# vlongle/pixie

Measured on NVIDIA H100. Metric: unet_voxels_per_s, higher is better.
Workload: dtype fp16e5 (U-Net, fp32 accumulate) + f32 (MPM)

## Files before the change

### pixie_b200/csrc/conv3d_igemm.cu

```cuda
#include "conv3d_igemm.cuh"
#include "ptx.cuh"

#include <algorithm>
#include <cmath>
#include <cstdio>
#include <cstring>

#include <cuda_fp8.h>

namespace pixie {

using namespace ptx;

namespace {

constexpr int kMaxWStages = 4;
constexpr int kMaxSStages = 8;
constexpr int kConsumerWarps = 8;
constexpr int kProducerWarp = 8;

struct SmemCtrl {
    uint64_t wfull[kMaxWStages];
    uint64_t wempty[kMaxWStages];
    uint64_t sfull[kMaxSStages];
    uint64_t sempty[kMaxSStages];
    int abort_flag;
};

constexpr int kCtlBarrierBytes = 512;
constexpr int kCmChunk = 16;
constexpr int kCmStageLd = 68;
constexpr int kCmStageFloats = kCmChunk * kCmStageLd;
constexpr int kStatsMaxC = 256;

struct TileCoord {
    int nb, d0, h0, w0, n0, ph_begin, ph_end, split, tde;
};

__device__ __forceinline__ TileCoord decode_tile(const ConvKernelParams& p, int wi) {
    TileCoord t;
    unsigned rest = (unsigned)wi;
    if (p.split_k == 1) {
        t.split = 0; t.ph_begin = 0; t.ph_end = p.n_phases;
    } else {
        const unsigned sk = (unsigned)p.split_k;
        t.split = (int)(rest % sk);
        rest /= sk;
        t.ph_begin = (int)(((unsigned)t.split * (unsigned)p.n_phases) / sk);
// ... 62 lines not shown
};

struct PendingStages {
    int s = -1, w = -1;
    __device__ __forceinline__ void release(SmemCtrl* ctl, int lane) {
        if (lane == 0) {
            if (s >= 0) mbar_arrive(&ctl->sempty[s]);
            if (w >= 0) mbar_arrive(&ctl->wempty[w]);
        }
        s = -1; w = -1;
    }
};

struct ConvStats {
    float* rows;
    int nb = -1;
    double tot_s = 0.0, tot_q = 0.0;

    __device__ __forceinline__ void flush(const ConvKernelParams& p, int lane) {
        if (p.stats_scalar) {
#pragma unroll
            for (int off = 16; off >= 1; off >>= 1) {
                tot_s += __shfl_xor_sync(0xffffffffu, tot_s, off);
                tot_q += __shfl_xor_sync(0xffffffffu, tot_q, off);
            }
            if (lane == 0) {
                atomicAdd(p.stats + (size_t)nb * p.Cout * 2, tot_s);
                atomicAdd(p.stats + (size_t)nb * p.Cout * 2 + 1, tot_q);
            }
            tot_s = 0.0; tot_q = 0.0;
            return;
        }
        asm volatile("bar.sync 1, 256;" ::: "memory");
        for (int ch = threadIdx.x; ch < p.Cout; ch += 256) {
            atomicAdd(p.stats + ((size_t)nb * p.Cout + ch) * 2, (double)rows[ch]);
            atomicAdd(p.stats + ((size_t)nb * p.Cout + ch) * 2 + 1, (double)rows[p.stats_ld + ch]);
            rows[ch] = 0.f;
            rows[p.stats_ld + ch] = 0.f;
        }
        asm volatile("bar.sync 1, 256;" ::: "memory");
    }
    __device__ __forceinline__ void enter(const ConvKernelParams& p, int item_nb, int lane) {
        if (nb != item_nb) {
            if (nb >= 0) flush(p, lane);
            nb = item_nb;
        }
    }
};

struct ConvSmem {
    uint8_t* w;
    uint8_t* s;
    SmemCtrl* ctl;
    float* stage;
    float* stats;
};

__device__ __forceinline__ ConvSmem conv_prologue(const ConvKernelParams& p, int stage_floats, int n_threads) {
    extern __shared__ __align__(1024) uint8_t smem_raw[];
    uint8_t* smem = reinterpret_cast<uint8_t*>(
        (reinterpret_cast<uintptr_t>(smem_raw) + 1023) & ~static_cast<uintptr_t>(1023));
    ConvSmem m;
    m.w = smem;
    m.s = smem + (size_t)p.w_stages * p.w_stage_bytes;
    m.ctl = reinterpret_cast<SmemCtrl*>(m.s + (size_t)p.s_stages * p.s_stage_bytes);
    m.stage = reinterpret_cast<float*>(reinterpret_cast<uint8_t*>(m.ctl) + kCtlBarrierBytes);
    m.stats = m.stage + stage_floats;
    const bool smem_misaligned = (p.smem_slack == 0) && (smem != smem_raw);

    if (threadIdx.x == 0) {
        for (int i = 0; i < kMaxWStages; ++i) { mbar_init(&m.ctl->wfull[i], 1); mbar_init(&m.ctl->wempty[i], kConsumerWarps); }
        for (int i = 0; i < kMaxSStages; ++i) { mbar_init(&m.ctl->sfull[i], 1); mbar_init(&m.ctl->sempty[i], kConsumerWarps); }
        m.ctl->abort_flag = smem_misaligned ? 1 : 0;
        fence_barrier_init();
    }
    if ((threadIdx.x >> 5) == kProducerWarp && (threadIdx.x & 31) == 0) {
        for (int i = 0; i < kConvMaxSrc; ++i) prefetch_tmap(&p.tmA[i]);
        prefetch_tmap(&p.tmB);
    }
    if (p.stats != nullptr && !p.stats_scalar)
        for (int i = threadIdx.x; i < 2 * p.stats_ld; i += n_threads) m.stats[i] = 0.f;
    __syncthreads();
    return m;
}

__device__ __forceinline__ void conv_report_abort(const ConvKernelParams& p, const SmemCtrl* ctl) {
    __syncthreads();
    if (threadIdx.x == 0 && ctl->abort_flag && p.err_flag) atomicExch(p.err_flag, 1 + (int)blockIdx.x);
}

template <int BN, int TD>
__device__ __forceinline__ int issue_slab(float (&acc)[TD][BN / 2], uint32_t a_addr, uint32_t w_addr, int pl, int d_min, int d_max,
                                          int n_kd, int n_kh, int TW, bool f8) {
    int groups = 0;
#pragma unroll
    for (int d = 0; d < TD; ++d) {
// ... 44 lines not shown
                    wring.advance(p.w_stages);
                }
                ok = mbar_wait(&ctl->sempty[sring.stage], sring.parity ^ 1, abort_flag);
                if (!ok) break;
                if (elect_one()) {
                    mbar_expect_tx(&ctl->sfull[sring.stage], slab_bytes);
                    tma_load_5d(s_smem + (size_t)sring.stage * p.s_stage_bytes, tm, &ctl->sfull[sring.stage], (int)P.c0, cw, ch,
                                cd + pl * p.stride, t.nb);
                }
                sring.advance(p.s_stages);
            }
        }
    }
}

}

template <int BN, int TD>
__global__ void __launch_bounds__(kConvThreads, 1)
conv3d_igemm_kernel(const __grid_constant__ ConvKernelParams p) {
    const ConvSmem sm = conv_prologue(p, 0, kConvThreads);
    SmemCtrl* ctl = sm.ctl;
    volatile int* abort_flag = &ctl->abort_flag;
    const int warp = threadIdx.x >> 5;
    const int lane = threadIdx.x & 31;
    const int total_items = conv_work_items(p.NB, p.tiles_d, p.tiles_h, p.tiles_w, p.n_tiles, p.split_k);
    const bool do_stats = p.stats != nullptr;
    const bool scalar_stats = do_stats && p.stats_scalar;

    if (warp == kProducerWarp) {
        produce_tiles<kWholePhase>(p, ctl, sm.w, sm.s, abort_flag, total_items);
    } else {
        const int g = warp >> 2, wq = warp & 3;
        float acc[TD][BN / 2];
        RingPos wring, sring;
        const uint32_t w_base0 = smem_u32(sm.w), s_base0 = smem_u32(sm.s) + (uint32_t)(g * 64 * 128);
        bool ok = true;
        const long long DHW = (long long)p.D * p.H * p.W;
        ConvStats stats{sm.stats};
        int th2[2], tw2[2];
#pragma unroll
        for (int r2 = 0; r2 < 2; ++r2) {
            const int r = g * 64 + wq * 16 + (lane >> 2) + 8 * r2;
            th2[r2] = r / p.TW; tw2[r2] = r % p.TW;
        }
        const int cq = (lane & 3) * 2;

        for (int wi = blockIdx.x; wi < total_items && ok; wi += gridDim.x) {
            const TileCoord t = decode_tile(p, wi);
#pragma unroll
            for (int d = 0; d < TD; ++d)
#pragma unroll
                for (int j = 0; j < BN / 2; ++j) acc[d][j] = 0.f;
            PendingStages pend;
// ... 113 lines not shown
                            const int ch = t.n0 + j8 * 8 + cq + e;
                            if (lane < 4 && ch < p.Cout) {
                                atomicAdd(stats.rows + ch, s);
                                atomicAdd(stats.rows + p.stats_ld + ch, q2);
                            }
                        }
                }
            }
        }
        if (do_stats && stats.nb >= 0 && ok) stats.flush(p, lane);
    }

    conv_report_abort(p, ctl);
}

template <int NV>
__global__ void __launch_bounds__(kConvCmThreads, 1)
conv3d_igemm_cm_kernel(const __grid_constant__ ConvKernelParams p) {
    constexpr int TW = NV == 64 ? 8 : 16;
    const ConvSmem sm = conv_prologue(p, 2 * kCmStageFloats, kConvCmThreads);
    SmemCtrl* ctl = sm.ctl;
    volatile int* abort_flag = &ctl->abort_flag;
    const int warp = threadIdx.x >> 5;
    const int lane = threadIdx.x & 31;
    const int total_items = conv_work_items(p.NB, p.tiles_d, p.tiles_h, p.tiles_w, p.n_tiles, p.split_k);
    const bool do_stats = p.stats != nullptr;
    const bool scalar_stats = do_stats && p.stats_scalar;

    if (warp >= kProducerWarp) {
        setmaxnreg_dec<NV == 256 ? 40 : 56>();
        if (warp == kProducerWarp) produce_tiles<1>(p, ctl, sm.w, sm.s, abort_flag, total_items);
    } else {
        setmaxnreg_inc<NV == 256 ? 232 : 216>();
        const int g = warp >> 2, wq = warp & 3, wt = threadIdx.x & 127;
        float acc[NV / 2];
        RingPos wring, sring;
        const uint32_t w_base0 = smem_u32(sm.w), s_base0 = smem_u32(sm.s);
        bool ok = true;
        ConvStats stats{sm.stats};
        const int q4 = wt & 15, vr = wt >> 4;
        float* stage = sm.stage + g * kCmStageFloats;

        for (int wi = blockIdx.x; wi < total_items && ok; wi += gridDim.x) {
            const TileCoord t = decode_tile(p, wi);
#pragma unroll
            for (int j = 0; j < NV / 2; ++j) acc[j] = 0.f;
            const bool has_plane = g < t.tde;
            PendingStages pend;
            int prev_f8 = -1;
            for (int ph = t.ph_begin; ph < t.ph_end && ok; ++ph) {
                const ConvPhase P = p.phases[ph];
                const int n_kd = P.n_kd, n_kh = P.n_kh;
                const bool f8 = P.f8 != 0;
                if (prev_f8 >= 0 && prev_f8 != (int)f8) wgmma_wait<0>();
                prev_f8 = (int)f8;
                const int w0 = wring.stage;
                const int nplanes = t.tde + n_kd - 1;
                for (int pl = 0; pl < nplanes && ok; ++pl) {
                    if (pl < n_kd) {
                        ok = mbar_wait(&ctl->wfull[wring.stage], wring.parity, abort_flag);
                        if (!ok) break;
                        wring.advance(p.w_stages);
                    }
                    ok = mbar_wait(&ctl->sfull[sring.stage], sring.parity, abort_flag);
                    if (!ok) break;
                    const int kd = pl - g;
                    int groups = 0;
                    if (has_plane && kd >= 0 && kd < n_kd) {
                        int wsk = w0 + kd;
                        if (wsk >= p.w_stages) wsk -= p.w_stages;
                        const uint32_t w_addr = w_base0 + (uint32_t)(wsk * p.w_stage_bytes);
                        const uint32_t s_addr = s_base0 + (uint32_t)(sring.stage * p.s_stage_bytes);
                        for (int kh = 0; kh < n_kh; ++kh) {
                            const uint32_t a = w_addr + (uint32_t)(conv_wtile(0, 1, kh, 0) * 64 * 128);
                            const uint32_t b = s_addr + (uint32_t)(kh * TW * 128);
                            if (f8) mma_block<NV, true>(acc, a, b);
                            else mma_block<NV, false>(acc, a, b);
                            ++groups;
                        }
                    }
                    wgmma_wait_n(groups);
                    pend.release(ctl, lane);
                    pend.s = sring.stage;
                    const int kd_done = pl - t.tde + 1;
                    if (kd_done >= 0) {
                        pend.w = w0 + kd_done;
                        if (pend.w >= p.w_stages) pend.w -= p.w_stages;
                    }
                    sring.advance(p.s_stages);
                }
            }
            wgmma_wait<0>();
            pend.release(ctl, lane);
#pragma unroll
            for (int j = 0; j < NV / 2; ++j) fence_operand(acc[j]);
            if (!ok) break;

            if (do_stats) stats.enter(p, t.nb, lane);
            if (!has_plane) continue;
            const bool first_split = (t.split == 0);
            const int ch = t.n0 + 4 * q4;
            const bool ch_ok = ch < p.Cout;
            float4 bias4 = make_float4(0.f, 0.f, 0.f, 0.f);
            if (first_split && p.bias != nullptr && ch_ok)
                bias4 = make_float4(__ldg(p.bias + ch), __ldg(p.bias + ch + 1), __ldg(p.bias + ch + 2), __ldg(p.bias + ch + 3));
            const bool use_res = first_split && p.residual != nullptr;
            const long long plane_base = ((long long)t.nb * p.D + t.d0 + g) * p.H;
            float st_s[4] = {0.f, 0.f, 0.f, 0.f}, st_q[4] = {0.f, 0.f, 0.f, 0.f};
#pragma unroll
            for (int c = 0; c < NV / kCmChunk; ++c) {
#pragma unroll
                for (int jj = 0; jj < kCmChunk / 8; ++jj)
#pragma unroll
                    for (int r2 = 0; r2 < 2; ++r2)
#pragma unroll
                        for (int e = 0; e < 2; ++e) {
                            const int row = wq * 16 + (lane >> 2) + 8 * r2, v = jj * 8 + (lane & 3) * 2 + e;
                            stage[v * kCmStageLd + row] = acc[(c * (kCmChunk / 8) + jj) * 4 + r2 * 2 + e];
                        }
                asm volatile("bar.sync %0, 128;" ::"r"(2 + g) : "memory");
#pragma unroll
                for (int k = 0; k < kCmChunk / 8; ++k) {
                    const int v = vr + 8 * k, vt = c * kCmChunk + v;
                    const int hh = t.h0 + vt / TW, ww = t.w0 + vt % TW;
                    float4 x = *reinterpret_cast<const float4*>(stage + v * kCmStageLd + 4 * q4);
                    if (ch_ok && hh < p.H && ww < p.W) {
                        const long long base = ((plane_base + hh) * p.W + ww) * p.out_ld + p.out_c0 + ch;
                        x.x += bias4.x; x.y += bias4.y; x.z += bias4.z; x.w += bias4.w;
                        if (use_res) {
                            const float4 rv = __ldg(reinterpret_cast<const float4*>(p.residual + base));
                            x.x += rv.x; x.y += rv.y; x.z += rv.z; x.w += rv.w;
                        }
                        if (p.atomic_out) red_add_v4(p.out + base, x.x, x.y, x.z, x.w);
                        else *reinterpret_cast<float4*>(p.out + base) = x;
                        st_s[0] += x.x; st_s[1] += x.y; st_s[2] += x.z; st_s[3] += x.w;
                        st_q[0] = fmaf(x.x, x.x, st_q[0]); st_q[1] = fmaf(x.y, x.y, st_q[1]);
                        st_q[2] = fmaf(x.z, x.z, st_q[2]); st_q[3] = fmaf(x.w, x.w, st_q[3]);
                    }
                }
                asm volatile("bar.sync %0, 128;" ::"r"(2 + g) : "memory");
            }
            if (do_stats) {
                if (scalar_stats) {
                    stats.tot_s += (double)(st_s[0] + st_s[1] + st_s[2] + st_s[3]);
                    stats.tot_q += (double)(st_q[0] + st_q[1] + st_q[2] + st_q[3]);
                } else {
#pragma unroll
                    for (int i = 0; i < 4; ++i) {
                        st_s[i] += __shfl_xor_sync(0xffffffffu, st_s[i], 16);
                        st_q[i] += __shfl_xor_sync(0xffffffffu, st_q[i], 16);
                    }
                    if (lane < 16 && ch_ok) {
#pragma unroll
                        for (int i = 0; i < 4; ++i) {
                            atomicAdd(stats.rows + ch + i, st_s[i]);
                            atomicAdd(stats.rows + p.stats_ld + ch + i, st_q[i]);
                        }
                    }
                }
            }
        }
        if (do_stats && stats.nb >= 0 && ok) stats.flush(p, lane);
    }

    conv_report_abort(p, ctl);
}


int conv_k_total(const ConvDesc& d) {
    int k = 0;
    for (const auto& s : d.segs) k += s.ks * s.ks * s.ks * d.srcs[s.src].C;
    return k;
}

struct SrcSlot { int src; int n_kh; };
// ... 144 lines not shown
        CUresult r = enc(&p.tmA[i], CU_TENSOR_MAP_DATA_TYPE_FLOAT16, 5, (void*)s.ptr, gdim, gstr, box, estr,
                         CU_TENSOR_MAP_INTERLEAVE_NONE, CU_TENSOR_MAP_SWIZZLE_128B,
                         CU_TENSOR_MAP_L2_PROMOTION_L2_256B, CU_TENSOR_MAP_FLOAT_OOB_FILL_NONE);
        if (r != CUDA_SUCCESS) { snprintf(err, errlen, "cuTensorMapEncodeTiled(A%zu) failed: %d", i, (int)r); return 1; }
    }
    for (size_t i = slots.size(); i < (size_t)kConvMaxSrc; ++i) p.tmA[i] = p.tmA[0];
    return 0;
}

int conv_plan_retarget(const ConvDesc& d, ConvPlan& plan, char* err, int errlen) {
    PFN_encodeTiled enc = get_encode_fn();
    if (!enc) { snprintf(err, errlen, "cuTensorMapEncodeTiled unavailable"); return 1; }
    return encode_a_maps(d, plan.p, enc, err, errlen);
}

static const char* cm_geometry(const ConvDesc& d, int sms, int max_kh, ConvKernelParams& p) {
    int nv = d.nv;
    if (nv && nv != 64 && nv != 128 && nv != 256) return "bad nv";
    if (!nv) {
        double best = -1.0;
        for (int v : {256, 128, 64}) {
            if (v != 64 && d.W < 16) continue;
            const int tw = v == 64 ? 8 : 16, th = v / tw;
            const int tx = (d.W + tw - 1) / tw, ty = (d.H + th - 1) / th;
            const long long tiles = conv_work_items(d.NB, (d.D + 1) / 2, ty, tx, (d.Cout_pad + 63) / 64, 1);
            const long long rounds = (tiles + sms - 1) / sms;
            const double sc = (double)tiles / (double)(rounds * sms) * (double)d.W * d.H / (double)(tx * tw * ty * th) *
                              std::pow(0.93, v == 256 ? 0 : v == 128 ? 1 : 2);
            if (sc > best) { best = sc; nv = v; }
        }
    }
    p.TW = nv == 64 ? 8 : 16;
    p.TH = nv / p.TW;
    p.TD = 2;
    p.block_n = 64;
    p.w_stage_bytes = max_kh * p.block_n * 128;
    return nullptr;
}

static bool cm_stages(const ConvKernelParams& p, int max_kd, int avail, int& ws, int& ss) {
    ws = std::max(2, max_kd);
    if (ws * p.w_stage_bytes + 2 * p.s_stage_bytes > avail) return false;
    ss = std::min(std::min(kMaxSStages, 6), (avail - ws * p.w_stage_bytes) / p.s_stage_bytes);
    ws = std::min(kMaxWStages, (avail - ss * p.s_stage_bytes) / p.w_stage_bytes);
    return true;
}
// ... 54 lines not shown
    int max_taps = 1, max_kh = 1, max_kd = 1;
    bool any3 = false;
    for (const auto& P : phases) {
        max_taps = std::max(max_taps, P.n_kh * P.n_kd);
        max_kh = std::max(max_kh, (int)P.n_kh);
        max_kd = std::max(max_kd, (int)P.n_kd);
        any3 |= (P.n_kh == 3);
    }

    int dev = 0, sms = 132;
    cudaGetDevice(&dev);
    cudaDeviceGetAttribute(&sms, cudaDevAttrMultiProcessorCount, dev);

    plan.channel_major = d.Cout >= 64 && d.Cout % 4 == 0 && !d.out_planar && out_ld % 4 == 0 && d.out_c0 % 4 == 0 &&
                         reinterpret_cast<uintptr_t>(d.out) % 16 == 0 && reinterpret_cast<uintptr_t>(d.residual) % 16 == 0;
    const char* bad = plan.channel_major ? cm_geometry(d, sms, max_kh, p) : vm_geometry(d, sms, any3, max_taps, p);
    if (bad) return fail(bad);
    p.n_tiles = (d.Cout_pad + p.block_n - 1) / p.block_n;
    p.tiles_w = (d.W + p.TW - 1) / p.TW;
    p.tiles_h = (d.H + p.TH - 1) / p.TH;
    p.tiles_d = (d.D + p.TD - 1) / p.TD;

    const int items = conv_work_items(d.NB, p.tiles_d, p.tiles_h, p.tiles_w, p.n_tiles, 1);
    int split = d.split_k;
    if (split <= 0) {
        split = 1;
        while (items * split < 120 && split * 2 <= p.n_phases && split < 64) split *= 2;
    }
    split = std::max(1, std::min(split, p.n_phases));
    if ((long long)p.n_phases * (split + 1) >= (1ll << 31)) return fail("too many phases for the split-K bookkeeping");
    p.split_k = split;
    p.atomic_out = split > 1;
    plan.needs_zero = split > 1;

    for (size_t i = 0; i < slots.size(); ++i) p.slab_rows[i] = p.TW * (p.TH + slots[i].n_kh - 1);
    int max_rows = 0;
    for (size_t i = 0; i < slots.size(); ++i) max_rows = std::max(max_rows, p.slab_rows[i]);
    p.s_stage_bytes = max_rows * 128;
    plan.fused_stats = d.stats != nullptr && split == 1 && d.Cout <= kStatsMaxC && !d.out_planar;
    p.stats_ld = (d.Cout + 31) / 32 * 32;
    const int stats_bytes = plan.fused_stats ? 2 * p.stats_ld * 4 : 0;
    const int ctl_core = kCtlBarrierBytes + (plan.channel_major ? 2 * kCmStageFloats * 4 : 0) + stats_bytes;
    auto plan_stages = [&](int slack, int& ws, int& ss) {
        const int avail = 227 * 1024 - ctl_core - slack;
        return plan.channel_major ? cm_stages(p, max_kd, avail, ws, ss) : vm_stages(p, avail, ws, ss);
    };
    int ws1 = 0, ss1 = 0, ws0 = 0, ss0 = 0;
    const bool ok1 = plan_stages(1024, ws1, ss1), ok0 = plan_stages(0, ws0, ss0);
    if (!ok0) return fail("tile does not fit in shared memory");
    if (ok1 && ws1 >= ws0 && ss1 >= ss0) { p.smem_slack = 1024; p.w_stages = ws1; p.s_stages = ss1; }
    else { p.smem_slack = 0; p.w_stages = ws0; p.s_stages = ss0; }
    const int ctl_bytes = ctl_core + p.smem_slack;
    plan.smem_bytes = p.w_stages * p.w_stage_bytes + p.s_stages * p.s_stage_bytes + ctl_bytes;

    if (encode_a_maps(d, p, enc, err, errlen)) return 1;
    {
// ... 10 lines not shown

    if (cudaMalloc(&plan.d_phases, phases.size() * sizeof(ConvPhase)) != cudaSuccess) return fail("cudaMalloc phases");
    cudaMemcpy(plan.d_phases, phases.data(), phases.size() * sizeof(ConvPhase), cudaMemcpyHostToDevice);
    p.phases = plan.d_phases;

    p.bias = d.bias; p.residual = d.residual; p.out = d.out;
    p.out_ld = out_ld; p.out_c0 = d.out_c0; p.out_planar = d.out_planar;
    p.err_flag = d_err_flag;
    p.stats = plan.fused_stats ? d.stats : nullptr;
    p.stats_scalar = d.stats_scalar ? 1 : 0;
    plan.out_item_bytes = d.out_planar ? (size_t)d.Cout * d.D * d.H * d.W * 4
                                       : (size_t)d.D * d.H * d.W * p.out_ld * 4;

    plan.grid = std::min(items * split, sms);

    plan.kernel = plan.channel_major ? conv_cm_kernel_for(p.TH * p.TW) : conv_kernel_for(p.block_n, p.TD);
    plan.threads = plan.channel_major ? kConvCmThreads : kConvThreads;
    if (cudaFuncSetAttribute(plan.kernel, cudaFuncAttributeMaxDynamicSharedMemorySize, 227 * 1024) != cudaSuccess)
        return fail("cudaFuncSetAttribute(max dynamic smem)");
    return 0;
}

void conv_plan_destroy(ConvPlan& plan) {
    if (plan.d_phases) cudaFree(plan.d_phases);
    plan.d_phases = nullptr;
}

int conv_plan_launch(const ConvPlan& plan, int nb, cudaStream_t stream) {
    if (nb < 1 || nb > plan.p.NB) return (int)cudaErrorInvalidValue;
    ConvKernelParams p = plan.p;
    p.NB = nb;
// ... 8 lines not shown
```

### pixie_b200/csrc/conv3d_igemm.cuh

```cuda
#pragma once
#include <cuda.h>
#include <cuda_runtime.h>
#include <cuda_fp16.h>
#include <cstdint>
#include <vector>

namespace pixie {

constexpr int kConvMaxSrc = 8;
constexpr int kF8Shift = 6;
constexpr int kConvThreads = 288;
constexpr int kConvCmThreads = 384;

struct ConvPhase {
    int8_t src;
    int8_t dw;
    int8_t dh0;
    int8_t dd0;
    int8_t n_kh;
    int8_t n_kd;
    int16_t c0;
    int32_t wtile_base;
    int32_t f8;
};
// ... 53 lines not shown
    struct Seg { int src; int ks; int wlo = 0; int f8 = 0; int lo = 0; };
    std::vector<ConvSrc> srcs;
    std::vector<Seg> segs;
    const __half* weights = nullptr;
    int Cout_pad = 0;
    const float* bias = nullptr;
    const float* residual = nullptr;
    float* out = nullptr;
    int out_ld = 0, out_c0 = 0, out_planar = 0;
    double* stats = nullptr;
    bool stats_scalar = false;
    int split_k = 1;
    int block_n = 0;
    int td = 0;
    int nv = 0;
};

int conv_k_total(const ConvDesc& d);

std::vector<ConvPhase> conv_build_phases(const ConvDesc& d);

void conv_pack_weights(const ConvDesc& d, const std::vector<const float*>& seg_weights,
                       const std::vector<int>& seg_cin_real, std::vector<__half>& packed);

struct ConvPlan {
    ConvKernelParams p{};
    ConvPhase* d_phases = nullptr;
    ConvKernelFn kernel = nullptr;
    bool channel_major = false;
    int threads = 0;
    int grid = 0;
    int smem_bytes = 0;
    bool needs_zero = false;
    bool fused_stats = false;
    size_t out_item_bytes = 0;
};

int conv_plan_create(const ConvDesc& d, int* d_err_flag, ConvPlan& plan, char* err, int errlen);
void conv_plan_destroy(ConvPlan& plan);
int conv_plan_launch(const ConvPlan& plan, int nb, cudaStream_t stream);
int conv_plan_retarget(const ConvDesc& d, ConvPlan& plan, char* err, int errlen);
}
```

### pixie_b200/csrc/ptx.cuh

```cuda
#pragma once
#include <cstdint>
#include <cuda_runtime.h>

namespace pixie {
namespace ptx {

__device__ __forceinline__ uint32_t smem_u32(const void* p) {
    return static_cast<uint32_t>(__cvta_generic_to_shared(p));
}

__device__ __forceinline__ bool elect_one() {
    uint32_t pred = 0;
    asm volatile(
        "{\n\t"
        ".reg .pred P;\n\t"
        "elect.sync _|P, 0xffffffff;\n\t"
        "selp.u32 %0, 1, 0, P;\n\t"
        "}\n"
        : "=r"(pred));
    return pred != 0;
}

__device__ __forceinline__ void mbar_init(uint64_t* bar, uint32_t count) {
    asm volatile("mbarrier.init.shared::cta.b64 [%0], %1;" ::"r"(smem_u32(bar)), "r"(count));
// ... 146 lines not shown
        : "+f"(d[0]), "+f"(d[1]), "+f"(d[2]), "+f"(d[3]), "+f"(d[4]), "+f"(d[5]), "+f"(d[6]), "+f"(d[7]), "+f"(d[8]), "+f"(d[9]), "+f"(d[10]), "+f"(d[11]), "+f"(d[12]), "+f"(d[13]), "+f"(d[14]), "+f"(d[15]), "+f"(d[16]), "+f"(d[17]), "+f"(d[18]), "+f"(d[19]), "+f"(d[20]), "+f"(d[21]), "+f"(d[22]), "+f"(d[23]), "+f"(d[24]), "+f"(d[25]), "+f"(d[26]), "+f"(d[27]), "+f"(d[28]), "+f"(d[29]), "+f"(d[30]), "+f"(d[31]), "+f"(d[32]), "+f"(d[33]), "+f"(d[34]), "+f"(d[35]), "+f"(d[36]), "+f"(d[37]), "+f"(d[38]), "+f"(d[39]), "+f"(d[40]), "+f"(d[41]), "+f"(d[42]), "+f"(d[43]), "+f"(d[44]), "+f"(d[45]), "+f"(d[46]), "+f"(d[47]), "+f"(d[48]), "+f"(d[49]), "+f"(d[50]), "+f"(d[51]), "+f"(d[52]), "+f"(d[53]), "+f"(d[54]), "+f"(d[55]), "+f"(d[56]), "+f"(d[57]), "+f"(d[58]), "+f"(d[59]), "+f"(d[60]), "+f"(d[61]), "+f"(d[62]), "+f"(d[63])
        : "l"(da), "l"(db), "r"(1));
}
__device__ __forceinline__ void wgmma_e5m2_n256(float* d, uint64_t da, uint64_t db) {
    asm volatile(
        "{\n\t.reg .pred p;\n\tsetp.ne.b32 p, %130, 0;\n\t"
        "wgmma.mma_async.sync.aligned.m64n256k32.f32.e5m2.e5m2 "
        "{%0, %1, %2, %3, %4, %5, %6, %7, %8, %9, %10, %11, %12, %13, %14, %15, %16, %17, %18, %19, %20, %21, %22, %23, %24, %25, %26, %27, %28, %29, %30, %31, %32, %33, %34, %35, %36, %37, %38, %39, %40, %41, %42, %43, %44, %45, %46, %47, %48, %49, %50, %51, %52, %53, %54, %55, %56, %57, %58, %59, %60, %61, %62, %63, %64, %65, %66, %67, %68, %69, %70, %71, %72, %73, %74, %75, %76, %77, %78, %79, %80, %81, %82, %83, %84, %85, %86, %87, %88, %89, %90, %91, %92, %93, %94, %95, %96, %97, %98, %99, %100, %101, %102, %103, %104, %105, %106, %107, %108, %109, %110, %111, %112, %113, %114, %115, %116, %117, %118, %119, %120, %121, %122, %123, %124, %125, %126, %127}, %128, %129, p, 1, 1;\n\t}\n"
        : "+f"(d[0]), "+f"(d[1]), "+f"(d[2]), "+f"(d[3]), "+f"(d[4]), "+f"(d[5]), "+f"(d[6]), "+f"(d[7]), "+f"(d[8]), "+f"(d[9]), "+f"(d[10]), "+f"(d[11]), "+f"(d[12]), "+f"(d[13]), "+f"(d[14]), "+f"(d[15]), "+f"(d[16]), "+f"(d[17]), "+f"(d[18]), "+f"(d[19]), "+f"(d[20]), "+f"(d[21]), "+f"(d[22]), "+f"(d[23]), "+f"(d[24]), "+f"(d[25]), "+f"(d[26]), "+f"(d[27]), "+f"(d[28]), "+f"(d[29]), "+f"(d[30]), "+f"(d[31]), "+f"(d[32]), "+f"(d[33]), "+f"(d[34]), "+f"(d[35]), "+f"(d[36]), "+f"(d[37]), "+f"(d[38]), "+f"(d[39]), "+f"(d[40]), "+f"(d[41]), "+f"(d[42]), "+f"(d[43]), "+f"(d[44]), "+f"(d[45]), "+f"(d[46]), "+f"(d[47]), "+f"(d[48]), "+f"(d[49]), "+f"(d[50]), "+f"(d[51]), "+f"(d[52]), "+f"(d[53]), "+f"(d[54]), "+f"(d[55]), "+f"(d[56]), "+f"(d[57]), "+f"(d[58]), "+f"(d[59]), "+f"(d[60]), "+f"(d[61]), "+f"(d[62]), "+f"(d[63]), "+f"(d[64]), "+f"(d[65]), "+f"(d[66]), "+f"(d[67]), "+f"(d[68]), "+f"(d[69]), "+f"(d[70]), "+f"(d[71]), "+f"(d[72]), "+f"(d[73]), "+f"(d[74]), "+f"(d[75]), "+f"(d[76]), "+f"(d[77]), "+f"(d[78]), "+f"(d[79]), "+f"(d[80]), "+f"(d[81]), "+f"(d[82]), "+f"(d[83]), "+f"(d[84]), "+f"(d[85]), "+f"(d[86]), "+f"(d[87]), "+f"(d[88]), "+f"(d[89]), "+f"(d[90]), "+f"(d[91]), "+f"(d[92]), "+f"(d[93]), "+f"(d[94]), "+f"(d[95]), "+f"(d[96]), "+f"(d[97]), "+f"(d[98]), "+f"(d[99]), "+f"(d[100]), "+f"(d[101]), "+f"(d[102]), "+f"(d[103]), "+f"(d[104]), "+f"(d[105]), "+f"(d[106]), "+f"(d[107]), "+f"(d[108]), "+f"(d[109]), "+f"(d[110]), "+f"(d[111]), "+f"(d[112]), "+f"(d[113]), "+f"(d[114]), "+f"(d[115]), "+f"(d[116]), "+f"(d[117]), "+f"(d[118]), "+f"(d[119]), "+f"(d[120]), "+f"(d[121]), "+f"(d[122]), "+f"(d[123]), "+f"(d[124]), "+f"(d[125]), "+f"(d[126]), "+f"(d[127])
        : "l"(da), "l"(db), "r"(1));
}
template <int N>
__device__ __forceinline__ void setmaxnreg_dec() { asm volatile("setmaxnreg.dec.sync.aligned.u32 %0;" ::"n"(N)); }
template <int N>
__device__ __forceinline__ void setmaxnreg_inc() { asm volatile("setmaxnreg.inc.sync.aligned.u32 %0;" ::"n"(N)); }


__device__ __forceinline__ void cp_async_16(void* smem_dst, const void* gmem_src) {
    asm volatile("cp.async.cg.shared.global [%0], [%1], 16;" ::"r"(smem_u32(smem_dst)), "l"(gmem_src) : "memory");
}
__device__ __forceinline__ void cp_async_commit() { asm volatile("cp.async.commit_group;" ::: "memory"); }
template <int N>
__device__ __forceinline__ void cp_async_wait() { asm volatile("cp.async.wait_group %0;" ::"n"(N) : "memory"); }

__device__ __forceinline__ void red_add_v2(float* addr, float a, float b) {
    asm volatile("red.global.add.v2.f32 [%0], {%1, %2};" ::"l"(addr), "f"(a), "f"(b) : "memory");
}
__device__ __forceinline__ void red_add_v4(float* addr, float a, float b, float c, float d) {
    asm volatile("red.global.add.v4.f32 [%0], {%1, %2, %3, %4};" ::"l"(addr), "f"(a), "f"(b),
                 "f"(c), "f"(d)
// ... 16 lines not shown
```

Measured before the change: 16.02 million.

## Add ping-pong warpgroup schedule for channel-major conv3d implicit GEMM

Adds a channel-major conv kernel in which the two consumer warpgroups alternate work items. Each accumulates both depth planes of a 128-voxel tile, and named barriers hand over the turn so one group's epilogue overlaps the other's WGMMA mainloop. The mainloop, epilogue chunking and stats code are factored into shared helpers, and stats get per-group smem rows and barriers. The host geometry picker scores the ping-pong option with a penalty factor, and split-K is disabled for it. The cost is more register pressure (two accumulators) and extra synchronization complexity.

```diff
diff --git a/pixie_b200/csrc/conv3d_igemm.cu b/pixie_b200/csrc/conv3d_igemm.cu
--- a/pixie_b200/csrc/conv3d_igemm.cu
+++ b/pixie_b200/csrc/conv3d_igemm.cu
@@ -32,6 +32,7 @@
 constexpr int kCmStageLd = 68;
 constexpr int kCmStageFloats = kCmChunk * kCmStageLd;
 constexpr int kStatsMaxC = 256;
+constexpr double kPingPongGain = 0.75;
 
 struct TileCoord {
     int nb, d0, h0, w0, n0, ph_begin, ph_end, split, tde;
@@ -124,6 +125,7 @@
 
 struct ConvStats {
     float* rows;
+    int bar, n_thr, tid;
     int nb = -1;
     double tot_s = 0.0, tot_q = 0.0;
 
@@ -141,14 +143,14 @@
             tot_s = 0.0; tot_q = 0.0;
             return;
         }
-        asm volatile("bar.sync 1, 256;" ::: "memory");
-        for (int ch = threadIdx.x; ch < p.Cout; ch += 256) {
+        named_bar_sync(bar, n_thr);
+        for (int ch = tid; ch < p.Cout; ch += n_thr) {
             atomicAdd(p.stats + ((size_t)nb * p.Cout + ch) * 2, (double)rows[ch]);
             atomicAdd(p.stats + ((size_t)nb * p.Cout + ch) * 2 + 1, (double)rows[p.stats_ld + ch]);
             rows[ch] = 0.f;
             rows[p.stats_ld + ch] = 0.f;
         }
-        asm volatile("bar.sync 1, 256;" ::: "memory");
+        named_bar_sync(bar, n_thr);
     }
     __device__ __forceinline__ void enter(const ConvKernelParams& p, int item_nb, int lane) {
         if (nb != item_nb) {
@@ -166,7 +168,8 @@
     float* stats;
 };
 
-__device__ __forceinline__ ConvSmem conv_prologue(const ConvKernelParams& p, int stage_floats, int n_threads) {
+__device__ __forceinline__ ConvSmem conv_prologue(const ConvKernelParams& p, int stage_floats, int n_threads,
+                                                  int consumer_warps = kConsumerWarps, int stats_sets = 1) {
     extern __shared__ __align__(1024) uint8_t smem_raw[];
     uint8_t* smem = reinterpret_cast<uint8_t*>(
         (reinterpret_cast<uintptr_t>(smem_raw) + 1023) & ~static_cast<uintptr_t>(1023));
@@ -179,8 +182,8 @@
     const bool smem_misaligned = (p.smem_slack == 0) && (smem != smem_raw);
 
     if (threadIdx.x == 0) {
-        for (int i = 0; i < kMaxWStages; ++i) { mbar_init(&m.ctl->wfull[i], 1); mbar_init(&m.ctl->wempty[i], kConsumerWarps); }
-        for (int i = 0; i < kMaxSStages; ++i) { mbar_init(&m.ctl->sfull[i], 1); mbar_init(&m.ctl->sempty[i], kConsumerWarps); }
+        for (int i = 0; i < kMaxWStages; ++i) { mbar_init(&m.ctl->wfull[i], 1); mbar_init(&m.ctl->wempty[i], consumer_warps); }
+        for (int i = 0; i < kMaxSStages; ++i) { mbar_init(&m.ctl->sfull[i], 1); mbar_init(&m.ctl->sempty[i], consumer_warps); }
         m.ctl->abort_flag = smem_misaligned ? 1 : 0;
         fence_barrier_init();
     }
@@ -189,7 +192,7 @@
         prefetch_tmap(&p.tmB);
     }
     if (p.stats != nullptr && !p.stats_scalar)
-        for (int i = threadIdx.x; i < 2 * p.stats_ld; i += n_threads) m.stats[i] = 0.f;
+        for (int i = threadIdx.x; i < 2 * p.stats_ld * stats_sets; i += n_threads) m.stats[i] = 0.f;
     __syncthreads();
     return m;
 }
@@ -264,6 +267,171 @@
     }
 }
 
+
+
+template <int NV, int NP>
+__device__ __forceinline__ bool cm_mainloop(const ConvKernelParams& p, SmemCtrl* ctl, volatile int* abort_flag,
+                                            const TileCoord& t, float (&acc)[NP][NV / 2], int d_first, uint32_t w_base0,
+                                            uint32_t s_base0, RingPos& wring, RingPos& sring, PendingStages& pend, int lane) {
+    constexpr int TW = NV == 64 ? 8 : 16;
+#pragma unroll
+    for (int d = 0; d < NP; ++d)
+#pragma unroll
+        for (int j = 0; j < NV / 2; ++j) acc[d][j] = 0.f;
+    bool ok = true;
+    int prev_f8 = -1;
+    for (int ph = t.ph_begin; ph < t.ph_end && ok; ++ph) {
+        const ConvPhase P = p.phases[ph];
+        const int n_kd = P.n_kd, n_kh = P.n_kh;
+        const bool f8 = P.f8 != 0;
+        if (prev_f8 >= 0 && prev_f8 != (int)f8) wgmma_wait<0>();
+        prev_f8 = (int)f8;
+        const int w0 = wring.stage;
+        const int nplanes = t.tde + n_kd - 1;
+        for (int pl = 0; pl < nplanes && ok; ++pl) {
+            if (pl < n_kd) {
+                ok = mbar_wait(&ctl->wfull[wring.stage], wring.parity, abort_flag);
+                if (!ok) break;
+                wring.advance(p.w_stages);
+            }
+            ok = mbar_wait(&ctl->sfull[sring.stage], sring.parity, abort_flag);
+            if (!ok) break;
+            int groups = 0;
+#pragma unroll
+            for (int d = 0; d < NP; ++d) {
+                const int kd = pl - d_first - d;
+                if (d_first + d < t.tde && kd >= 0 && kd < n_kd) {
+                    int wsk = w0 + kd;
+                    if (wsk >= p.w_stages) wsk -= p.w_stages;
+                    const uint32_t w_addr = w_base0 + (uint32_t)(wsk * p.w_stage_bytes);
+                    const uint32_t s_addr = s_base0 + (uint32_t)(sring.stage * p.s_stage_bytes);
+                    for (int kh = 0; kh < n_kh; ++kh) {
+                        const uint32_t a = w_addr + (uint32_t)(conv_wtile(0, 1, kh, 0) * 64 * 128);
+                        const uint32_t b = s_addr + (uint32_t)(kh * TW * 128);
+                        if (f8) mma_block<NV, true>(acc[d], a, b);
+                        else mma_block<NV, false>(acc[d], a, b);
+                        ++groups;
+                    }
+                }
+            }
+            wgmma_wait_n(groups);
+            pend.release(ctl, lane);
+            pend.s = sring.stage;
+            const int kd_done = pl - t.tde + 1;
+            if (kd_done >= 0) {
+                pend.w = w0 + kd_done;
+                if (pend.w >= p.w_stages) pend.w -= p.w_stages;
+            }
+            sring.advance(p.s_stages);
+        }
+    }
+    return ok;
+}
+
+constexpr int kCmChunkRows = kCmChunk / 8;
+struct CmChunk {
+    long long base[kCmChunkRows];
+    bool ok[kCmChunkRows];
+    float4 rv[kCmChunkRows];
+};
+
+template <int NV>
+__device__ __forceinline__ CmChunk cm_chunk(const ConvKernelParams& p, const TileCoord& t, int d, int c, int wt, bool use_res) {
+    constexpr int TW = NV == 64 ? 8 : 16;
+    const int ch = t.n0 + 4 * (wt & 15), vr = wt >> 4;
+    const bool ch_ok = ch < p.Cout;
+    const long long plane_base = ((long long)t.nb * p.D + t.d0 + d) * p.H;
+    CmChunk k;
+#pragma unroll
+    for (int r = 0; r < kCmChunkRows; ++r) {
+        const int vt = c * kCmChunk + vr + 8 * r;
+        const int hh = t.h0 + vt / TW, ww = t.w0 + vt % TW;
+        k.ok[r] = ch_ok && hh < p.H && ww < p.W;
+        k.base[r] = ((plane_base + hh) * p.W + ww) * p.out_ld + p.out_c0 + ch;
+        k.rv[r] = make_float4(0.f, 0.f, 0.f, 0.f);
+    }
+    if (use_res) {
+#pragma unroll
+        for (int r = 0; r < kCmChunkRows; ++r)
+            if (k.ok[r]) k.rv[r] = __ldg(reinterpret_cast<const float4*>(p.residual + k.base[r]));
+    }
+    return k;
+}
+
+template <int NV, bool kAhead>
+__device__ __forceinline__ void cm_store_plane(const ConvKernelParams& p, const TileCoord& t, int d, const float (&acc)[NV / 2],
+                                               CmChunk cur, float* stage, int bar, int wt, float4 bias4, bool use_res,
+                                               float (&st_s)[4], float (&st_q)[4]) {
+    const int lane = wt & 31, wq = wt >> 5, q4 = wt & 15, vr = wt >> 4;
+#pragma unroll
+    for (int c = 0; c < NV / kCmChunk; ++c) {
+        CmChunk next;
+        if (kAhead && c + 1 < NV / kCmChunk) next = cm_chunk<NV>(p, t, d, c + 1, wt, use_res);
+        if (!kAhead && c > 0) cur = cm_chunk<NV>(p, t, d, c, wt, use_res);
+#pragma unroll
+        for (int jj = 0; jj < kCmChunk / 8; ++jj)
+#pragma unroll
+            for (int r2 = 0; r2 < 2; ++r2)
+#pragma unroll
+                for (int e = 0; e < 2; ++e) {
+                    const int row = wq * 16 + (lane >> 2) + 8 * r2, v = jj * 8 + (lane & 3) * 2 + e;
+                    stage[v * kCmStageLd + row] = acc[(c * (kCmChunk / 8) + jj) * 4 + r2 * 2 + e];
+                }
+        named_bar_sync(bar, 128);
+#pragma unroll
+        for (int r = 0; r < kCmChunkRows; ++r) {
+            float4 x = *reinterpret_cast<const float4*>(stage + (vr + 8 * r) * kCmStageLd + 4 * q4);
+            if (cur.ok[r]) {
+                x.x += bias4.x; x.y += bias4.y; x.z += bias4.z; x.w += bias4.w;
+                if (use_res) { x.x += cur.rv[r].x; x.y += cur.rv[r].y; x.z += cur.rv[r].z; x.w += cur.rv[r].w; }
+                if (p.atomic_out) red_add_v4(p.out + cur.base[r], x.x, x.y, x.z, x.w);
+                else *reinterpret_cast<float4*>(p.out + cur.base[r]) = x;
+                st_s[0] += x.x; st_s[1] += x.y; st_s[2] += x.z; st_s[3] += x.w;
+                st_q[0] = fmaf(x.x, x.x, st_q[0]); st_q[1] = fmaf(x.y, x.y, st_q[1]);
+                st_q[2] = fmaf(x.z, x.z, st_q[2]); st_q[3] = fmaf(x.w, x.w, st_q[3]);
+            }
+        }
+        named_bar_sync(bar, 128);
+        if (kAhead && c + 1 < NV / kCmChunk) cur = next;
+    }
+}
+
+__device__ __forceinline__ float4 cm_bias4(const ConvKernelParams& p, const TileCoord& t, int wt) {
+    const int ch = t.n0 + 4 * (wt & 15);
+    if (t.split != 0 || p.bias == nullptr || ch >= p.Cout) return make_float4(0.f, 0.f, 0.f, 0.f);
+    return make_float4(__ldg(p.bias + ch), __ldg(p.bias + ch + 1), __ldg(p.bias + ch + 2), __ldg(p.bias + ch + 3));
+}
+
+__device__ __forceinline__ void cm_add_stats(const ConvKernelParams& p, ConvStats& stats, const TileCoord& t, int wt,
+                                             float (&st_s)[4], float (&st_q)[4]) {
+    if (p.stats_scalar) {
+        stats.tot_s += (double)(st_s[0] + st_s[1] + st_s[2] + st_s[3]);
+        stats.tot_q += (double)(st_q[0] + st_q[1] + st_q[2] + st_q[3]);
+        return;
+    }
+#pragma unroll
+    for (int i = 0; i < 4; ++i) {
+        st_s[i] += __shfl_xor_sync(0xffffffffu, st_s[i], 16);
+        st_q[i] += __shfl_xor_sync(0xffffffffu, st_q[i], 16);
+    }
+    const int ch = t.n0 + 4 * (wt & 15);
+    if ((wt & 31) < 16 && ch < p.Cout) {
+#pragma unroll
+        for (int i = 0; i < 4; ++i) {
+            atomicAdd(stats.rows + ch + i, st_s[i]);
+            atomicAdd(stats.rows + p.stats_ld + ch + i, st_q[i]);
+        }
+    }
+}
+
+__device__ __forceinline__ void cm_skip_item(const ConvKernelParams& p, const TileCoord& t, RingPos& wring, RingPos& sring) {
+    for (int ph = t.ph_begin; ph < t.ph_end; ++ph) {
+        const int n_kd = p.phases[ph].n_kd;
+        for (int u = 0; u < n_kd; ++u) wring.advance(p.w_stages);
+        for (int pl = 0; pl < t.tde + n_kd - 1; ++pl) sring.advance(p.s_stages);
+    }
+}
+
 }
 
 template <int BN, int TD>
@@ -287,7 +455,7 @@
         const uint32_t w_base0 = smem_u32(sm.w), s_base0 = smem_u32(sm.s) + (uint32_t)(g * 64 * 128);
         bool ok = true;
         const long long DHW = (long long)p.D * p.H * p.W;
-        ConvStats stats{sm.stats};
+        ConvStats stats{sm.stats, 1, 256, (int)threadIdx.x};
         int th2[2], tw2[2];
 #pragma unroll
         for (int r2 = 0; r2 < 2; ++r2) {
@@ -431,10 +599,10 @@
     conv_report_abort(p, ctl);
 }
 
+
 template <int NV>
 __global__ void __launch_bounds__(kConvCmThreads, 1)
 conv3d_igemm_cm_kernel(const __grid_constant__ ConvKernelParams p) {
-    constexpr int TW = NV == 64 ? 8 : 16;
     const ConvSmem sm = conv_prologue(p, 2 * kCmStageFloats, kConvCmThreads);
     SmemCtrl* ctl = sm.ctl;
     volatile int* abort_flag = &ctl->abort_flag;
@@ -442,140 +610,100 @@
     const int lane = threadIdx.x & 31;
     const int total_items = conv_work_items(p.NB, p.tiles_d, p.tiles_h, p.tiles_w, p.n_tiles, p.split_k);
     const bool do_stats = p.stats != nullptr;
-    const bool scalar_stats = do_stats && p.stats_scalar;
 
     if (warp >= kProducerWarp) {
         setmaxnreg_dec<NV == 256 ? 40 : 56>();
         if (warp == kProducerWarp) produce_tiles<1>(p, ctl, sm.w, sm.s, abort_flag, total_items);
     } else {
         setmaxnreg_inc<NV == 256 ? 232 : 216>();
-        const int g = warp >> 2, wq = warp & 3, wt = threadIdx.x & 127;
-        float acc[NV / 2];
+        const int g = warp >> 2, wt = threadIdx.x & 127;
+        float acc[1][NV / 2];
         RingPos wring, sring;
         const uint32_t w_base0 = smem_u32(sm.w), s_base0 = smem_u32(sm.s);
         bool ok = true;
-        ConvStats stats{sm.stats};
-        const int q4 = wt & 15, vr = wt >> 4;
+        ConvStats stats{sm.stats, 1, 256, (int)threadIdx.x};
         float* stage = sm.stage + g * kCmStageFloats;
 
         for (int wi = blockIdx.x; wi < total_items && ok; wi += gridDim.x) {
             const TileCoord t = decode_tile(p, wi);
-#pragma unroll
-            for (int j = 0; j < NV / 2; ++j) acc[j] = 0.f;
-            const bool has_plane = g < t.tde;
             PendingStages pend;
-            int prev_f8 = -1;
-            for (int ph = t.ph_begin; ph < t.ph_end && ok; ++ph) {
-                const ConvPhase P = p.phases[ph];
-                const int n_kd = P.n_kd, n_kh = P.n_kh;
-                const bool f8 = P.f8 != 0;
-                if (prev_f8 >= 0 && prev_f8 != (int)f8) wgmma_wait<0>();
-                prev_f8 = (int)f8;
-                const int w0 = wring.stage;
-                const int nplanes = t.tde + n_kd - 1;
-                for (int pl = 0; pl < nplanes && ok; ++pl) {
-                    if (pl < n_kd) {
-                        ok = mbar_wait(&ctl->wfull[wring.stage], wring.parity, abort_flag);
-                        if (!ok) break;
-                        wring.advance(p.w_stages);
-                    }
-                    ok = mbar_wait(&ctl->sfull[sring.stage], sring.parity, abort_flag);
-                    if (!ok) break;
-                    const int kd = pl - g;
-                    int groups = 0;
-                    if (has_plane && kd >= 0 && kd < n_kd) {
-                        int wsk = w0 + kd;
-                        if (wsk >= p.w_stages) wsk -= p.w_stages;
-                        const uint32_t w_addr = w_base0 + (uint32_t)(wsk * p.w_stage_bytes);
-                        const uint32_t s_addr = s_base0 + (uint32_t)(sring.stage * p.s_stage_bytes);
-                        for (int kh = 0; kh < n_kh; ++kh) {
-                            const uint32_t a = w_addr + (uint32_t)(conv_wtile(0, 1, kh, 0) * 64 * 128);
-                            const uint32_t b = s_addr + (uint32_t)(kh * TW * 128);
-                            if (f8) mma_block<NV, true>(acc, a, b);
-                            else mma_block<NV, false>(acc, a, b);
-                            ++groups;
-                        }
-                    }
-                    wgmma_wait_n(groups);
-                    pend.release(ctl, lane);
-                    pend.s = sring.stage;
-                    const int kd_done = pl - t.tde + 1;
-                    if (kd_done >= 0) {
-                        pend.w = w0 + kd_done;
-                        if (pend.w >= p.w_stages) pend.w -= p.w_stages;
-                    }
-                    sring.advance(p.s_stages);
-                }
-            }
+            ok = cm_mainloop<NV, 1>(p, ctl, abort_flag, t, acc, g, w_base0, s_base0, wring, sring, pend, lane);
+            const bool use_res = t.split == 0 && p.residual != nullptr;
+            const CmChunk first = cm_chunk<NV>(p, t, g, 0, wt, use_res && ok && g < t.tde);
             wgmma_wait<0>();
             pend.release(ctl, lane);
 #pragma unroll
-            for (int j = 0; j < NV / 2; ++j) fence_operand(acc[j]);
+            for (int j = 0; j < NV / 2; ++j) fence_operand(acc[0][j]);
             if (!ok) break;
 
             if (do_stats) stats.enter(p, t.nb, lane);
-            if (!has_plane) continue;
-            const bool first_split = (t.split == 0);
-            const int ch = t.n0 + 4 * q4;
-            const bool ch_ok = ch < p.Cout;
-            float4 bias4 = make_float4(0.f, 0.f, 0.f, 0.f);
-            if (first_split && p.bias != nullptr && ch_ok)
-                bias4 = make_float4(__ldg(p.bias + ch), __ldg(p.bias + ch + 1), __ldg(p.bias + ch + 2), __ldg(p.bias + ch + 3));
-            const bool use_res = first_split && p.residual != nullptr;
-            const long long plane_base = ((long long)t.nb * p.D + t.d0 + g) * p.H;
+            if (g >= t.tde) continue;
             float st_s[4] = {0.f, 0.f, 0.f, 0.f}, st_q[4] = {0.f, 0.f, 0.f, 0.f};
-#pragma unroll
-            for (int c = 0; c < NV / kCmChunk; ++c) {
-#pragma unroll
-                for (int jj = 0; jj < kCmChunk / 8; ++jj)
-#pragma unroll
-                    for (int r2 = 0; r2 < 2; ++r2)
-#pragma unroll
-                        for (int e = 0; e < 2; ++e) {
-                            const int row = wq * 16 + (lane >> 2) + 8 * r2, v = jj * 8 + (lane & 3) * 2 + e;
-                            stage[v * kCmStageLd + row] = acc[(c * (kCmChunk / 8) + jj) * 4 + r2 * 2 + e];
-                        }
-                asm volatile("bar.sync %0, 128;" ::"r"(2 + g) : "memory");
-#pragma unroll
-                for (int k = 0; k < kCmChunk / 8; ++k) {
-                    const int v = vr + 8 * k, vt = c * kCmChunk + v;
-                    const int hh = t.h0 + vt / TW, ww = t.w0 + vt % TW;
-                    float4 x = *reinterpret_cast<const float4*>(stage + v * kCmStageLd + 4 * q4);
-                    if (ch_ok && hh < p.H && ww < p.W) {
-                        const long long base = ((plane_base + hh) * p.W + ww) * p.out_ld + p.out_c0 + ch;
-                        x.x += bias4.x; x.y += bias4.y; x.z += bias4.z; x.w += bias4.w;
-                        if (use_res) {
-                            const float4 rv = __ldg(reinterpret_cast<const float4*>(p.residual + base));
-                            x.x += rv.x; x.y += rv.y; x.z += rv.z; x.w += rv.w;
-                        }
-                        if (p.atomic_out) red_add_v4(p.out + base, x.x, x.y, x.z, x.w);
-                        else *reinterpret_cast<float4*>(p.out + base) = x;
-                        st_s[0] += x.x; st_s[1] += x.y; st_s[2] += x.z; st_s[3] += x.w;
-                        st_q[0] = fmaf(x.x, x.x, st_q[0]); st_q[1] = fmaf(x.y, x.y, st_q[1]);
-                        st_q[2] = fmaf(x.z, x.z, st_q[2]); st_q[3] = fmaf(x.w, x.w, st_q[3]);
-                    }
-                }
-                asm volatile("bar.sync %0, 128;" ::"r"(2 + g) : "memory");
-            }
-            if (do_stats) {
-                if (scalar_stats) {
-                    stats.tot_s += (double)(st_s[0] + st_s[1] + st_s[2] + st_s[3]);
-                    stats.tot_q += (double)(st_q[0] + st_q[1] + st_q[2] + st_q[3]);
-                } else {
-#pragma unroll
-                    for (int i = 0; i < 4; ++i) {
-                        st_s[i] += __shfl_xor_sync(0xffffffffu, st_s[i], 16);
-                        st_q[i] += __shfl_xor_sync(0xffffffffu, st_q[i], 16);
-                    }
-                    if (lane < 16 && ch_ok) {
-#pragma unroll
-                        for (int i = 0; i < 4; ++i) {
-                            atomicAdd(stats.rows + ch + i, st_s[i]);
-                            atomicAdd(stats.rows + p.stats_ld + ch + i, st_q[i]);
-                        }
-                    }
-                }
-            }
+            cm_store_plane<NV, true>(p, t, g, acc[0], first, stage, 2 + g, wt, cm_bias4(p, t, wt), use_res, st_s, st_q);
+            if (do_stats) cm_add_stats(p, stats, t, wt, st_s, st_q);
+        }
+        if (do_stats && stats.nb >= 0 && ok) stats.flush(p, lane);
+    }
+
+    conv_report_abort(p, ctl);
+}
+
+constexpr int kCmTurnBar = 4;
+
+__global__ void __launch_bounds__(kConvCmThreads, 1)
+conv3d_igemm_cm_pingpong_kernel(const __grid_constant__ ConvKernelParams p) {
+    constexpr int NV = 128;
+    const ConvSmem sm = conv_prologue(p, 2 * kCmStageFloats, kConvCmThreads, kConsumerWarps / 2, 2);
+    SmemCtrl* ctl = sm.ctl;
+    volatile int* abort_flag = &ctl->abort_flag;
+    const int warp = threadIdx.x >> 5;
+    const int lane = threadIdx.x & 31;
+    const int total_items = conv_work_items(p.NB, p.tiles_d, p.tiles_h, p.tiles_w, p.n_tiles, p.split_k);
+    const bool do_stats = p.stats != nullptr;
+
+    if (warp >= kProducerWarp) {
+        setmaxnreg_dec<40>();
+        if (warp == kProducerWarp) produce_tiles<1>(p, ctl, sm.w, sm.s, abort_flag, total_items);
+    } else {
+        setmaxnreg_inc<232>();
+        const int g = warp >> 2, wt = threadIdx.x & 127;
+        float acc[2][NV / 2];
+        RingPos wring, sring;
+        const uint32_t w_base0 = smem_u32(sm.w), s_base0 = smem_u32(sm.s);
+        bool ok = true;
+        ConvStats stats{sm.stats + g * 2 * p.stats_ld, 2 + g, 128, wt};
+        float* stage = sm.stage + g * kCmStageFloats;
+
+        for (int k = 0, wi = blockIdx.x; wi < total_items; ++k, wi += gridDim.x) {
+            const TileCoord t = decode_tile(p, wi);
+            if ((k & 1) != g) {
+                cm_skip_item(p, t, wring, sring);
+                continue;
+            }
+            bool turn = true;
+            if (k > 0) {
+                if (*abort_flag) turn = false;
+                else named_bar_sync(kCmTurnBar + g, 256);
+            }
+            PendingStages pend;
+            ok = turn && cm_mainloop<NV, 2>(p, ctl, abort_flag, t, acc, 0, w_base0, s_base0, wring, sring, pend, lane);
+            if (wi + (int)gridDim.x < total_items) named_bar_arrive(kCmTurnBar + (g ^ 1), 256);
+            wgmma_wait<0>();
+            pend.release(ctl, lane);
+#pragma unroll
+            for (int d = 0; d < 2; ++d)
+#pragma unroll
+                for (int j = 0; j < NV / 2; ++j) fence_operand(acc[d][j]);
+            if (!ok) break;
+
+            if (do_stats) stats.enter(p, t.nb, lane);
+            const float4 bias4 = cm_bias4(p, t, wt);
+            const bool use_res = p.residual != nullptr;
+            float st_s[4] = {0.f, 0.f, 0.f, 0.f}, st_q[4] = {0.f, 0.f, 0.f, 0.f};
+            cm_store_plane<NV, false>(p, t, 0, acc[0], cm_chunk<NV>(p, t, 0, 0, wt, use_res), stage, 2 + g, wt, bias4, use_res, st_s, st_q);
+            if (t.tde > 1)
+                cm_store_plane<NV, false>(p, t, 1, acc[1], cm_chunk<NV>(p, t, 1, 0, wt, use_res), stage, 2 + g, wt, bias4, use_res, st_s, st_q);
+            if (do_stats) cm_add_stats(p, stats, t, wt, st_s, st_q);
         }
         if (do_stats && stats.nb >= 0 && ok) stats.flush(p, lane);
     }
@@ -750,22 +878,30 @@
     return encode_a_maps(d, plan.p, enc, err, errlen);
 }
 
-static const char* cm_geometry(const ConvDesc& d, int sms, int max_kh, ConvKernelParams& p) {
+static const char* cm_geometry(const ConvDesc& d, int sms, int max_kh, ConvKernelParams& p, bool& pingpong) {
     int nv = d.nv;
     if (nv && nv != 64 && nv != 128 && nv != 256) return "bad nv";
-    if (!nv) {
+    pingpong = d.pingpong == 1;
+    if (pingpong && ((nv && nv != 128) || d.W < 16)) return "the ping-pong schedule needs 8 x 16 voxel tiles";
+    if (pingpong && d.split_k > 1) return "the ping-pong schedule does not split K";
+    if (!nv && !pingpong) {
         double best = -1.0;
-        for (int v : {256, 128, 64}) {
-            if (v != 64 && d.W < 16) continue;
-            const int tw = v == 64 ? 8 : 16, th = v / tw;
+        for (int v : {256, 128, 64, -128}) {
+            const bool pp = v < 0;
+            const int nvv = pp ? -v : v;
+            if (nvv != 64 && d.W < 16) continue;
+            if (pp && (d.pingpong == 0 || d.split_k > 1)) continue;
+            const int tw = nvv == 64 ? 8 : 16, th = nvv / tw, workers = pp ? 2 * sms : sms;
             const int tx = (d.W + tw - 1) / tw, ty = (d.H + th - 1) / th;
             const long long tiles = conv_work_items(d.NB, (d.D + 1) / 2, ty, tx, (d.Cout_pad + 63) / 64, 1);
-            const long long rounds = (tiles + sms - 1) / sms;
-            const double sc = (double)tiles / (double)(rounds * sms) * (double)d.W * d.H / (double)(tx * tw * ty * th) *
-                              std::pow(0.93, v == 256 ? 0 : v == 128 ? 1 : 2);
-            if (sc > best) { best = sc; nv = v; }
-        }
-    }
+            if (pp && tiles < 2ll * workers) continue;
+            const long long rounds = (tiles + workers - 1) / workers;
+            const double sc = (double)tiles / (double)(rounds * workers) * (double)d.W * d.H / (double)(tx * tw * ty * th) *
+                              std::pow(0.93, nvv == 256 ? 0 : nvv == 128 ? 1 : 2) * (pp ? kPingPongGain : 1.0);
+            if (sc > best) { best = sc; nv = nvv; pingpong = pp; }
+        }
+    }
+    if (pingpong) nv = 128;
     p.TW = nv == 64 ? 8 : 16;
     p.TH = nv / p.TW;
     p.TD = 2;
@@ -850,7 +986,9 @@
 
     plan.channel_major = d.Cout >= 64 && d.Cout % 4 == 0 && !d.out_planar && out_ld % 4 == 0 && d.out_c0 % 4 == 0 &&
                          reinterpret_cast<uintptr_t>(d.out) % 16 == 0 && reinterpret_cast<uintptr_t>(d.residual) % 16 == 0;
-    const char* bad = plan.channel_major ? cm_geometry(d, sms, max_kh, p) : vm_geometry(d, sms, any3, max_taps, p);
+    if (d.pingpong == 1 && !plan.channel_major) return fail("the ping-pong schedule needs a channel-major output");
+    plan.pingpong = false;
+    const char* bad = plan.channel_major ? cm_geometry(d, sms, max_kh, p, plan.pingpong) : vm_geometry(d, sms, any3, max_taps, p);
     if (bad) return fail(bad);
     p.n_tiles = (d.Cout_pad + p.block_n - 1) / p.block_n;
     p.tiles_w = (d.W + p.TW - 1) / p.TW;
@@ -861,7 +999,7 @@
     int split = d.split_k;
     if (split <= 0) {
         split = 1;
-        while (items * split < 120 && split * 2 <= p.n_phases && split < 64) split *= 2;
+        while (!plan.pingpong && items * split < 120 && split * 2 <= p.n_phases && split < 64) split *= 2;
     }
     split = std::max(1, std::min(split, p.n_phases));
     if ((long long)p.n_phases * (split + 1) >= (1ll << 31)) return fail("too many phases for the split-K bookkeeping");
@@ -875,7 +1013,7 @@
     p.s_stage_bytes = max_rows * 128;
     plan.fused_stats = d.stats != nullptr && split == 1 && d.Cout <= kStatsMaxC && !d.out_planar;
     p.stats_ld = (d.Cout + 31) / 32 * 32;
-    const int stats_bytes = plan.fused_stats ? 2 * p.stats_ld * 4 : 0;
+    const int stats_bytes = plan.fused_stats ? 2 * p.stats_ld * 4 * (plan.pingpong ? 2 : 1) : 0;
     const int ctl_core = kCtlBarrierBytes + (plan.channel_major ? 2 * kCmStageFloats * 4 : 0) + stats_bytes;
     auto plan_stages = [&](int slack, int& ws, int& ss) {
         const int avail = 227 * 1024 - ctl_core - slack;
@@ -916,7 +1054,8 @@
 
     plan.grid = std::min(items * split, sms);
 
-    plan.kernel = plan.channel_major ? conv_cm_kernel_for(p.TH * p.TW) : conv_kernel_for(p.block_n, p.TD);
+    plan.kernel = plan.pingpong ? conv3d_igemm_cm_pingpong_kernel
+                  : plan.channel_major ? conv_cm_kernel_for(p.TH * p.TW) : conv_kernel_for(p.block_n, p.TD);
     plan.threads = plan.channel_major ? kConvCmThreads : kConvThreads;
     if (cudaFuncSetAttribute(plan.kernel, cudaFuncAttributeMaxDynamicSharedMemorySize, 227 * 1024) != cudaSuccess)
         return fail("cudaFuncSetAttribute(max dynamic smem)");
diff --git a/pixie_b200/csrc/conv3d_igemm.cuh b/pixie_b200/csrc/conv3d_igemm.cuh
--- a/pixie_b200/csrc/conv3d_igemm.cuh
+++ b/pixie_b200/csrc/conv3d_igemm.cuh
@@ -91,6 +91,7 @@
     int block_n = 0;
     int td = 0;
     int nv = 0;
+    int pingpong = -1;
 };
 
 int conv_k_total(const ConvDesc& d);
@@ -105,6 +106,7 @@
     ConvPhase* d_phases = nullptr;
     ConvKernelFn kernel = nullptr;
     bool channel_major = false;
+    bool pingpong = false;
     int threads = 0;
     int grid = 0;
     int smem_bytes = 0;
diff --git a/pixie_b200/csrc/ptx.cuh b/pixie_b200/csrc/ptx.cuh
--- a/pixie_b200/csrc/ptx.cuh
+++ b/pixie_b200/csrc/ptx.cuh
@@ -184,6 +184,8 @@
 __device__ __forceinline__ void setmaxnreg_dec() { asm volatile("setmaxnreg.dec.sync.aligned.u32 %0;" ::"n"(N)); }
 template <int N>
 __device__ __forceinline__ void setmaxnreg_inc() { asm volatile("setmaxnreg.inc.sync.aligned.u32 %0;" ::"n"(N)); }
+__device__ __forceinline__ void named_bar_sync(int id, int n) { asm volatile("bar.sync %0, %1;" ::"r"(id), "r"(n) : "memory"); }
+__device__ __forceinline__ void named_bar_arrive(int id, int n) { asm volatile("bar.arrive %0, %1;" ::"r"(id), "r"(n) : "memory"); }
 
 
 __device__ __forceinline__ void cp_async_16(void* smem_dst, const void* gmem_src) {
```

After: 16.18 million, median of 6. 1.01x the previous value.
